# twosixlabs/csl-gan

Hardware: AMD Instinct MI355X
Metric: images/sec/GPU CelebA DCResNet dp_mode=gc bs=128 at 1/2/4/8 MI355X (higher is better)
Workload: dtype f32; 1 GPU; CelebA DCResNet D-step: dp_mode=gc -gcm adaptive-pl -nms 32, WGAN-GP on mean samples, 3x64x64; compute_dtype=fp32_auto, storage_dtype=fp32, launch=hip_graph, batch_per_gpu=128, global_batch=128, parallelism=dp1, materialize=ghost, grad_sample_dtype=fp32, fuse_passes=True

## Files before the change

### csl_gan_amd/DCResNet_models.py

```python
import torch
import torch.nn.functional as F
from torch import nn

from . import functional as HF
from . import ops
from .models import Discriminator, Generator
from .nn import HipConv2d, HipGroupNormAct, HipLinear


class UpsampleConv(nn.Module):

    def __init__(self, in_ch, out_ch, filter_size, bias=True):
        super().__init__()
        self.conv = HipConv2d(in_ch, out_ch, filter_size, padding="same", bias=bias)

    def forward_shuffled(self, x_ps):
        return self.conv.forward_shuffled(x_ps)

    def forward(self, x):
        if x.is_cuda:
            if x.shape[1] % 4:
                raise NotImplementedError("UpsampleConv on HIP needs in_ch %% 4 == 0 (got %d)" % x.shape[1])
            return HF.nchw_view(self.forward_shuffled(HF.DepthToSpace.apply(HF.nhwc(x))))
        return self.conv(F.pixel_shuffle(torch.cat([x, x, x, x], 1), 2))
# ... 39 lines not shown
    from . import nn as hnn
    return (not torch.is_grad_enabled()) and x.is_cuda and x.dtype == torch.float32 and not ops.storage_bf16() and hnn._mask_recorder is None


def _norm_as_affine(norm, x, part, conv):
    if part is None or not ops.in_affine_ok(x, conv.weight.permute(0, 2, 3, 1), conv.stride[0], conv.padding[0]):
        return None
    N, H, W, C = x.shape
    sc, sh = ops.groupnorm_affine(part, norm.weight.detach(), norm.bias.detach(), norm.num_groups, norm.eps, N, H * W, C)
    return sc, sh, bool(norm.relu)


def _norm_act(bn, ch):
    return _BatchNormAct(ch) if bn else HipGroupNormAct(32, ch, relu=True)


class ResBlockUp(nn.Module):

    def __init__(self, in_ch, out_ch, filter_size, bn=True):
        super().__init__()
        self.shortcut = UpsampleConv(in_ch, out_ch, 1)
        self.bn1 = _norm_act(bn, in_ch)
        self.convUp = UpsampleConv(in_ch, out_ch, filter_size, bias=False)
        self.bn2 = _norm_act(bn, out_ch)
        self.conv = HipConv2d(out_ch, out_ch, filter_size, padding="same")

    def forward_nhwc(self, x):
        return self.forward_nhwc_parts(x)[0]

    def forward_nhwc_parts(self, x, x_part=None, next_norm=None):
        if x.shape[-1] % 4:
            raise NotImplementedError("ResBlockUp on HIP needs in_ch %% 4 == 0 (got %d)" % x.shape[-1])
        fuse = _gn_fusable(x)
        a_ps, x_ps = self.bn1.forward_shuffled(x, part=x_part) if x_part is not None else self.bn1.forward_shuffled(x)
        s = self.shortcut.forward_shuffled(x_ps)
        affine = None
        if fuse and isinstance(self.bn2, HipGroupNormAct):
            with ops.gn_partials(self.bn2.num_groups) as cell:
                o = self.convUp.forward_shuffled(a_ps)
            affine = _norm_as_affine(self.bn2, o, cell.part, self.conv)
            h = o if affine is not None else self.bn2.forward_nhwc(o, part=cell.part)
        else:
            h = self.bn2.forward_nhwc(self.convUp.forward_shuffled(a_ps))
        if fuse and isinstance(next_norm, HipGroupNormAct):
            with ops.gn_partials(next_norm.num_groups) as cell:
                out = self.conv.forward_nhwc(h, residual=s, in_affine=affine)
            return out, cell.part
        return self.conv.forward_nhwc(h, residual=s, in_affine=affine), None

    def forward(self, x):
        if x.is_cuda:
            return HF.nchw_view(self.forward_nhwc(HF.nhwc(x)))
        return self.conv(self.bn2(self.convUp(self.bn1(x)))) + self.shortcut(x)


class DCResNetGenerator(Generator):
    def __init__(self, channels, first_filter_size, **kwargs):
        super().__init__(**kwargs)
        self.first_filter_size = first_filter_size
        extra = self.n_classes if self.emb_mode == "concat" else 0
        self.linIn = HipLinear(self.z_dim + extra, first_filter_size ** 2 * channels[0])
        self.blocks = nn.ModuleList([ResBlockUp(a, b, 5, bn=self.bn) for a, b in zip(channels[:-1], channels[1:])])
        self.bn = _norm_act(self.bn, channels[-1])
        self.convOut = HipConv2d(channels[-1], self.out_ch, 3, padding="same", act=ops.ACT_TANH)

    def forward(self, z, y=None, out=None):
        f = self.first_filter_size
        x = self.linIn(self._condition(z, y)).reshape(z.size(0), -1, f, f)
# ... 70 lines not shown
```

### csl_gan_amd/_lib.py

```python
from __future__ import annotations

import ctypes as C
import os

_HERE = os.path.dirname(os.path.abspath(__file__))
LIB_PATH = os.environ.get("CSLGAN_LIB_PATH") or os.path.join(_HERE, "libcslgan_hip.so")
MAX_SEGS = 16
ABI_VERSION = 7

EXPORTS = [
    "cslgan_version", "cslgan_last_error", "cslgan_last_kernel", "cslgan_device_count",
    "cslgan_sample_sqnorm_f32", "cslgan_sample_sqnorm_bf16", "cslgan_clip_factors_f32", "cslgan_clip_accum_noise_f32",
    "cslgan_clip_accum_noise_bf16", "cslgan_conv2d_wgrad_grouped_bf16out_f32",
    "cslgan_l2_clip_rows_f32", "cslgan_row_l2norm_f32", "cslgan_row_l2norm_bwd_f32", "cslgan_mean_sample_f32",
    "cslgan_conv2d_fwd_f32", "cslgan_conv2d_fwd_x3_f32", "cslgan_conv2d_dgrad_f32", "cslgan_conv2d_wgrad_grouped_f32",
    "cslgan_conv2d_wgrad_scaled_f32", "cslgan_conv2d_wgrad_blocks_f32", "cslgan_conv2d_wgrad_sqnorm_gram_f32", "cslgan_conv2d_wgrad_skinny_f32", "cslgan_conv2d_s2_fwd_f32",
    "cslgan_conv2d_dgrad_x3_f32", "cslgan_conv2d_s2_fwd_x3_f32", "cslgan_u8_to_f32_nhwc", "cslgan_split_filter_x3_f32",
    "cslgan_depth_to_space_f32", "cslgan_fold_channels4_f32",
    "cslgan_bias_grad_grouped_f32", "cslgan_act_bwd_f32", "cslgan_groupnorm_act_f32", "cslgan_groupnorm_apply_parts_f32", "cslgan_groupnorm_affine_parts_f32", "cslgan_batchnorm_act_f32", "cslgan_batchnorm_eval_act_f32",
    "cslgan_norm_act_bwd_f32", "cslgan_norm_bwd_ws_floats",
    "cslgan_adam_step_f32", "cslgan_adam_step_dev_f32", "cslgan_adam_multi_f32",
    "cslgan_adaptive_clip_f32", "cslgan_segment_means_f32", "cslgan_segment_means_bwd_f32", "cslgan_dstep_stats_f32", "cslgan_grad_log_stats_f32",
    "cslgan_lerp_rows_f32", "cslgan_lipschitz_term_f32", "cslgan_lipschitz_term_bwd_f32",
    "cslgan_conv2d_fwd_bf16s", "cslgan_conv2d_dgrad_bf16s", "cslgan_conv2d_wgrad_grouped_bf16s", "cslgan_cast_f32_bf16", "cslgan_cast_bf16_f32",
    "cslgan_act_bwd_bf16", "cslgan_bias_grad_grouped_bf16", "cslgan_linear_k1_dgrad_bf16s", "cslgan_linear_k1_wgrad_bf16s",
    "cslgan_conv2d_c3_fwd_bf16out", "cslgan_conv2d_c3_wgrad_bf16gy", "cslgan_groupnorm_act_bf16s",
    "cslgan_conv2d_fwd_skinny_bf16in", "cslgan_conv2d_dgrad_skinny_bf16in", "cslgan_conv2d_wgrad_scaled_bf16s",
    "cslgan_latent_normal_f32", "cslgan_f32_to_u8",
    "cslgan_attack_trials", "cslgan_rank_counts", "cslgan_softmax_max_rows_f32",
    "cslgan_ovr_logreg_ws_floats", "cslgan_ovr_logreg_eval_f32", "cslgan_ovr_logreg_proba_f32",
    "cslgan_ovr_logreg_u8_ws_floats", "cslgan_ovr_logreg_eval_u8", "cslgan_ovr_logreg_proba_u8",
    "cslgan_ovr_mlp_u8_ws_floats", "cslgan_ovr_mlp_eval_u8", "cslgan_ovr_mlp_proba_u8",
    "cslgan_class_moments_u8", "cslgan_nb_score_gauss_u8", "cslgan_nb_score_bern_u8",
    "cslgan_nn_padded_dim", "cslgan_nn_prepare_u8", "cslgan_nn_min_i8", "cslgan_nn_count_i8",
    "cslgan_nn_kth_workspace_bytes", "cslgan_nn_kth_i8", "cslgan_nn_count_radius_i8",
]


class SegsT(C.Structure):
    _fields_ = [
        ("n_seg", C.c_int32), ("_pad", C.c_int32),
        ("inp", C.c_void_p * MAX_SEGS), ("out", C.c_void_p * MAX_SEGS), ("noise", C.c_void_p * MAX_SEGS),
        ("len", C.c_int64 * MAX_SEGS), ("row_stride", C.c_int64 * MAX_SEGS), ("rows", C.c_int64 * MAX_SEGS), ("call_counter", C.c_void_p),
    ]


MAX_CLIP_LAYERS, MAX_CLIP_JOBS = 32, 16


class AdaptiveClipT(C.Structure):
    _fields_ = [
        ("n_layers", C.c_int32), ("n_mat", C.c_int32), ("n_jobs", C.c_int32), ("_pad", C.c_int32),
# ... 30 lines not shown
    vp, i32, i64, f32, u64 = C.c_void_p, C.c_int, C.c_int64, C.c_float, C.c_uint64
    sig = {
        "cslgan_version": [],
        "cslgan_device_count": [],
        "cslgan_sample_sqnorm_f32": [C.POINTER(SegsT), i64, vp, vp],
        "cslgan_sample_sqnorm_bf16": [C.POINTER(SegsT), i64, vp, vp],
        "cslgan_clip_accum_noise_bf16": [C.POINTER(SegsT), i64, vp, i32, vp, u64, u64, f32, f32, vp],
        "cslgan_conv2d_wgrad_grouped_bf16out_f32": [C.POINTER(ConvT), vp, vp, i32, f32, vp, vp, vp],
        "cslgan_clip_factors_f32": [vp, i32, i64, vp, i32, f32, i64, vp, vp, vp],
        "cslgan_clip_accum_noise_f32": [C.POINTER(SegsT), i64, vp, i32, vp, u64, u64, f32, f32, vp],
        "cslgan_l2_clip_rows_f32": [vp, vp, i64, i64, f32, vp, vp],
        "cslgan_mean_sample_f32": [vp, i32, i32, i64, vp, vp, i64, f32, f32, u64, u64, vp, vp, vp],
        "cslgan_row_l2norm_f32": [vp, i64, i64, vp, vp],
        "cslgan_row_l2norm_bwd_f32": [vp, vp, vp, i64, i64, vp, vp],
        "cslgan_conv2d_fwd_f32": [C.POINTER(ConvT), vp, vp, vp, vp, i32, vp, vp],
        "cslgan_conv2d_fwd_x3_f32": [C.POINTER(ConvT), vp, vp, vp, i32, vp, vp, i32, vp, vp],
        "cslgan_conv2d_dgrad_f32": [C.POINTER(ConvT), vp, vp, vp, i32, vp, vp, vp],
        "cslgan_conv2d_dgrad_x3_f32": [C.POINTER(ConvT), vp, vp, vp, vp, i32, vp, vp, vp],
        "cslgan_norm_act_bwd_f32": [vp, vp, vp, vp, vp, i64, i64, i32, i32, f32, i32, vp, vp, vp, vp, vp],
        "cslgan_depth_to_space_f32": [vp, i32, i32, i32, i32, i32, vp, vp],
        "cslgan_fold_channels4_f32": [vp, i64, i32, i32, vp, vp],
        "cslgan_conv2d_wgrad_grouped_f32": [C.POINTER(ConvT), vp, vp, i32, f32, vp, vp, vp],
        "cslgan_conv2d_wgrad_scaled_f32": [C.POINTER(ConvT), vp, vp, vp, i32, f32, vp, vp],
        "cslgan_conv2d_wgrad_blocks_f32": [C.POINTER(ConvT), vp, vp, f32, i32, C.POINTER(C.c_int32), C.POINTER(vp), C.POINTER(vp), vp],
        "cslgan_conv2d_wgrad_sqnorm_gram_f32": [C.POINTER(ConvT), vp, vp, f32, vp, vp],
        "cslgan_conv2d_wgrad_skinny_f32": [C.POINTER(ConvT), vp, vp, f32, vp, i32, vp],
        "cslgan_conv2d_s2_fwd_f32": [C.POINTER(ConvT), vp, vp, vp, i32, vp, i32, vp, vp],
        "cslgan_conv2d_s2_fwd_x3_f32": [C.POINTER(ConvT), vp, vp, vp, vp, i32, vp, i32, vp, vp],
        "cslgan_bias_grad_grouped_f32": [vp, i32, i32, i32, i32, f32, vp, vp, vp],
        "cslgan_act_bwd_f32": [vp, vp, i64, f32, vp, vp],
        "cslgan_groupnorm_act_f32": [vp, vp, vp, i32, i32, i32, i32, f32, i32, vp, vp, i32, vp, vp, vp],
        "cslgan_groupnorm_affine_parts_f32": [vp, i32, vp, vp, i32, i32, i32, i32, f32, vp, vp, vp],
        "cslgan_groupnorm_apply_parts_f32": [vp, vp, vp, i32, i32, i32, i32, f32, i32, vp, i32, vp, vp, i32, vp, vp],
        "cslgan_batchnorm_act_f32": [vp, vp, vp, i64, i32, f32, i32, f32, vp, vp, vp, vp, i64, i32, vp, vp, vp],
        "cslgan_batchnorm_eval_act_f32": [vp, vp, vp, vp, vp, i64, i32, f32, i32, vp, vp, i64, i32, vp, vp],
        "cslgan_adam_step_f32": [vp, vp, vp, vp, i64, f32, f32, f32, f32, f32, i32, vp],
        "cslgan_adam_step_dev_f32": [vp, vp, vp, vp, i64, f32, f32, f32, f32, f32, vp, vp],
        "cslgan_adam_multi_f32": [i32, C.POINTER(vp), C.POINTER(vp), C.POINTER(vp), C.POINTER(vp), C.POINTER(i64), f32, f32, f32, f32, f32,
                                  i32, vp, vp],
        "cslgan_adaptive_clip_f32": [C.POINTER(AdaptiveClipT), i64, i64, i32, f32, i32, f32, i64, vp, vp, vp, vp, vp, vp],
        "cslgan_segment_means_f32": [vp, i32, C.POINTER(C.c_int32), C.POINTER(f32), vp, vp, vp],
        "cslgan_segment_means_bwd_f32": [vp, vp, i32, C.POINTER(C.c_int32), C.POINTER(f32), vp, vp],
        "cslgan_dstep_stats_f32": [vp, i32, vp, i32, vp, vp, vp, vp, vp],
        "cslgan_grad_log_stats_f32": [vp, i32, i64, i64, i32, vp, i32, f32, vp, vp, vp, vp, vp, vp],
        "cslgan_lerp_rows_f32": [vp, vp, vp, i64, i64, vp, vp],
        "cslgan_lipschitz_term_f32": [vp, i64, i64, i32, f32, vp, vp, vp, vp, vp],
        "cslgan_lipschitz_term_bwd_f32": [vp, vp, vp, vp, i64, i64, i32, f32, vp, vp],
        "cslgan_conv2d_fwd_bf16s": [C.POINTER(ConvT), vp, vp, vp, i32, vp, vp, i32, i32, vp, i32, vp],
        "cslgan_conv2d_dgrad_bf16s": [C.POINTER(ConvT), vp, vp, vp, i32, vp, vp, i32, vp],
        "cslgan_conv2d_wgrad_grouped_bf16s": [C.POINTER(ConvT), vp, vp, i32, f32, vp, i32, vp, vp],
        "cslgan_cast_f32_bf16": [vp, vp, i64, vp],
        "cslgan_u8_to_f32_nhwc": [vp, vp, i32, i32, i32, i32, C.c_float, C.c_float, vp, vp],
        "cslgan_split_filter_x3_f32": [vp, i32, i32, i32, vp, i32, vp],
        "cslgan_cast_bf16_f32": [vp, vp, i64, vp],
        "cslgan_act_bwd_bf16": [vp, vp, i64, f32, vp, vp],
        "cslgan_bias_grad_grouped_bf16": [vp, i32, i32, i32, i32, f32, vp, vp, vp],
        "cslgan_linear_k1_dgrad_bf16s": [vp, vp, vp, i32, i64, vp, vp],
        "cslgan_linear_k1_wgrad_bf16s": [vp, vp, vp, i32, i64, i32, f32, vp, vp, vp],
        "cslgan_conv2d_wgrad_scaled_bf16s": [C.POINTER(ConvT), vp, vp, vp, i32, f32, vp, vp],
        "cslgan_conv2d_c3_fwd_bf16out": [C.POINTER(ConvT), vp, vp, vp, i32, vp, vp],
        "cslgan_conv2d_c3_wgrad_bf16gy": [C.POINTER(ConvT), vp, vp, f32, vp, vp, vp],
        "cslgan_groupnorm_act_bf16s": [vp, i32, vp, vp, i32, i32, i32, i32, f32, i32, vp, vp, i32, vp, vp],
        "cslgan_conv2d_fwd_skinny_bf16in": [C.POINTER(ConvT), vp, vp, vp, i32, vp, vp],
        "cslgan_conv2d_dgrad_skinny_bf16in": [C.POINTER(ConvT), vp, vp, vp, i32, vp, vp],
        "cslgan_latent_normal_f32": [u64, u64, vp, i64, i32, vp, i32, i32, vp, vp],
        "cslgan_f32_to_u8": [vp, i64, f32, f32, vp, vp],
# ... 44 lines not shown
```

### csl_gan_amd/build.py

```python
import os
import subprocess
import sys

HERE = os.path.dirname(os.path.abspath(__file__))
CSRC = os.path.join(HERE, "csrc")
LIB = os.path.join(HERE, "libcslgan_hip.so")
SOURCES = ["clip_kernels.hip", "igemm_kc.hip", "igemm_halo.hip", "igemm_skinny.hip", "igemm_mc.hip", "igemm_wgh.hip", "igemm_bf16.hip", "igemm_x3.hip", "igemm_bf16s.hip", "conv_c3.hip", "linear_k1.hip", "conv1x1.hip", "gram_norm.hip", "pointwise_kernels.hip", "step_kernels.hip", "attack_kernels.hip", "logreg_kernels.hip", "mlp_kernels.hip", "nb_kernels.hip", "nn_kernels.hip"]
HEADERS = ["common.h", "igemm.h", "conv_classes.h", "device_prims.h", "kc_frame.h", "ovr_rows.h", os.path.join("..", "..", "include", "cslgan.h")]


def _newer_than(target, deps):
    if not os.path.exists(target):
        return True
    t = os.path.getmtime(target)
    return any(os.path.getmtime(d) > t for d in deps)


def build(force=False, verbose=False):
    force = force or os.environ.get("CSLGAN_FORCE_BUILD", "0") == "1"
    hipcc = os.environ.get("HIPCC", "/opt/rocm/bin/hipcc")
    headers = [os.path.join(CSRC, h) for h in HEADERS]
    objs = []
    procs = []
    os.makedirs(os.path.join(HERE, "build"), exist_ok=True)
    jobs = int(os.environ.get("CSLGAN_BUILD_JOBS", str(min(8, os.cpu_count() or 1))))
    pending = []
    for s in SOURCES:
        o = os.path.join(HERE, "build", s.replace(".hip", ".o"))
        objs.append(o)
        if force or _newer_than(o, [os.path.join(CSRC, s)] + headers):
            pending.append((s, o))
    while pending or procs:
        while pending and len(procs) < jobs:
            s, o = pending.pop(0)
            cmd = [hipcc, "--offload-arch=gfx950", "-O3", "-fPIC", "-std=c++17", "-Wall", "-Wno-unused-function",
                   "-c", os.path.join(CSRC, s), "-o", o]
            if verbose:
                print(" ".join(cmd))
            procs.append((s, subprocess.Popen(cmd, stdout=subprocess.PIPE, stderr=subprocess.STDOUT)))
        s, pr = procs.pop(0)
        out, _ = pr.communicate()
# ... 18 lines not shown
```

### csl_gan_amd/csrc/gram_norm.hip

```cpp
#include "common.h"
#include "device_prims.h"
#include "igemm.h"
#include "conv_classes.h"

namespace cslgan {


struct GramParams {
    const float* gy;
    const float* x;
    int N, H, W, C, K, PQ, Q, T, stride;
    int n1, n2;
    float alpha2;
    float* sq;
    signed char ty[IG_MAX_TAPS], tx[IG_MAX_TAPS];
};

constexpr int GR_LD = 36;

template <int TILES>
__global__ __launch_bounds__(256) void gram_sqnorm_kernel(const GramParams p) {
    constexpr int ROWS = TILES == 1 ? 128 : 64;
    constexpr int LPT = ROWS * 8 / 256;
    __shared__ __attribute__((aligned(16))) float As[2][ROWS * GR_LD];
    __shared__ float s_red[TILES == 1 ? 2 * 1024 : 4];

    const int tid = threadIdx.x;
    const int b = blockIdx.x;
    const int cpc = p.C >> 5;
    const int n_chunks = p.n1 + p.n2;
    const int n_iter = TILES == 1 ? (n_chunks + 3) / 4 : n_chunks;

    int l_pix[LPT], l_slot[LPT], l_py[LPT], l_px[LPT];
    const int j4 = (tid & 7) * 4;
#pragma unroll
    for (int i = 0; i < LPT; ++i) {
        const int row = (tid >> 3) + 32 * i;
        l_slot[i] = TILES == 1 ? row >> 5 : 0;
        l_pix[i] = TILES == 1 ? row & 31 : row;
        l_py[i] = l_pix[i] / p.Q;
        l_px[i] = l_pix[i] - l_py[i] * p.Q;
    }
    constexpr int DEPTH = TILES == 1 ? 4 : 6;
    float4 rg[DEPTH][LPT];
    auto load = [&](int it, float4* dst) {
#pragma unroll
        for (int i = 0; i < LPT; ++i) {
            const int c = TILES == 1 ? 4 * it + l_slot[i] : it;
            float4 v = make_float4(0.f, 0.f, 0.f, 0.f);
            if (l_pix[i] < p.PQ && c < n_chunks) {
                if (c < p.n1) {
                    v = *reinterpret_cast<const float4*>(p.gy + ((long long)b * p.PQ + l_pix[i]) * p.K + c * 32 + j4);
                } else {
                    const int c2 = c - p.n1;
                    const int t = c2 / cpc, cc = c2 - t * cpc;
                    const int iy = l_py[i] * p.stride + p.ty[t], ix = l_px[i] * p.stride + p.tx[t];
                    if ((unsigned)iy < (unsigned)p.H && (unsigned)ix < (unsigned)p.W)
                        v = *reinterpret_cast<const float4*>(p.x + (((long long)b * p.H + iy) * p.W + ix) * p.C + cc * 32 + j4);
// ... 34 lines not shown
                if (c < n_chunks) {
                    float4 af[4], bf[4];
#pragma unroll
                    for (int g = 0; g < 4; ++g) {
                        af[g] = *reinterpret_cast<const float4*>(&As[buf][rowA * GR_LD + 8 * g + 4 * h]);
                        bf[g] = *reinterpret_cast<const float4*>(&As[buf][rowB * GR_LD + 8 * g + 4 * h]);
                    }
                    if (c < p.n1) {
#pragma unroll
                        for (int g = 0; g < 4; ++g) {
                            acc1 = __builtin_amdgcn_mfma_f32_32x32x2f32(af[g].x, bf[g].x, acc1, 0, 0, 0);
                            acc1 = __builtin_amdgcn_mfma_f32_32x32x2f32(af[g].y, bf[g].y, acc1, 0, 0, 0);
                            acc1 = __builtin_amdgcn_mfma_f32_32x32x2f32(af[g].z, bf[g].z, acc1, 0, 0, 0);
                            acc1 = __builtin_amdgcn_mfma_f32_32x32x2f32(af[g].w, bf[g].w, acc1, 0, 0, 0);
                        }
                    } else {
#pragma unroll
                        for (int g = 0; g < 4; ++g) {
                            acc2 = __builtin_amdgcn_mfma_f32_32x32x2f32(af[g].x, bf[g].x, acc2, 0, 0, 0);
                            acc2 = __builtin_amdgcn_mfma_f32_32x32x2f32(af[g].y, bf[g].y, acc2, 0, 0, 0);
                            acc2 = __builtin_amdgcn_mfma_f32_32x32x2f32(af[g].z, bf[g].z, acc2, 0, 0, 0);
                            acc2 = __builtin_amdgcn_mfma_f32_32x32x2f32(af[g].w, bf[g].w, acc2, 0, 0, 0);
                        }
                    }
                }
                buf ^= 1;
            }
        }
    }
    __syncthreads();

    float prod = 0.f;
    if (TILES == 1) {
        for (int i = tid; i < 2 * 1024; i += 256) s_red[i] = 0.f;
        __syncthreads();
#pragma unroll
        for (int v = 0; v < 16; ++v) {
            const int row = (v & 3) + 8 * (v >> 2) + 4 * h;
            atomicAdd(&s_red[row * 32 + r], acc1[v]);
            atomicAdd(&s_red[1024 + row * 32 + r], acc2[v]);
        }
        __syncthreads();
        for (int i = tid; i < 1024; i += 256) prod = fmaf(s_red[i], s_red[1024 + i], prod);
        __syncthreads();
        const float tot = block_sum_256(prod, s_red);
        if (tid == 0) atomicAdd(p.sq + b, p.alpha2 * tot);
    } else {
#pragma unroll
        for (int v = 0; v < 16; ++v) prod = fmaf(acc1[v], acc2[v], prod);
        const float tot = block_sum_256(prod, s_red);
        if (tid == 0) atomicAdd(p.sq + b, p.alpha2 * tot);
    }
}



struct GramSmallParams {
    const float* gy;
    const float* x;
    int N, H, W, C, K, PQ, Q, T, s;
    float alpha2;
    float* sq;
    signed char tcls[IG_MAX_TAPS], tdy[IG_MAX_TAPS], tdx[IG_MAX_TAPS];
    int Hc[4], Wc[4];
};

__global__ __launch_bounds__(256) void gram_sqnorm_small_kernel(const GramSmallParams p) {
    __shared__ float XXs[4][16 * 17];
    __shared__ float G1s[4][16 * 17];
    __shared__ float s_red[4];
    const int tid = threadIdx.x, lane = tid & 63, wid = tid >> 6;
    const int b = blockIdx.x;
    const int row = lane & 15, q = lane >> 4;
    const int nc = p.s * p.s;
    f32x4 accx = {0.f, 0.f, 0.f, 0.f};
    if (wid < nc) {
        const int cy = wid / p.s, cx = wid - cy * p.s;
// ... 231 lines not shown
```

### csl_gan_amd/csrc/pointwise_kernels.hip

```cpp
#include "common.h"
#include "device_prims.h"

namespace cslgan {

__global__ void act_bwd_kernel(const float* __restrict__ g, const float* __restrict__ y, long long n, float slope,
                               float* __restrict__ out, int vec) {
    const long long stride = (long long)gridDim.x * blockDim.x;
    if (vec) {
        const long long n4 = n >> 2;
        const float4* g4 = reinterpret_cast<const float4*>(g);
        const float4* y4 = reinterpret_cast<const float4*>(y);
        float4* o4 = reinterpret_cast<float4*>(out);
        for (long long i = (long long)blockIdx.x * blockDim.x + threadIdx.x; i < n4; i += stride) {
            const float4 a = g4[i], b = y4[i];
            o4[i] = make_float4(b.x > 0.f ? a.x : slope * a.x, b.y > 0.f ? a.y : slope * a.y,
                                b.z > 0.f ? a.z : slope * a.z, b.w > 0.f ? a.w : slope * a.w);
        }
        for (long long i = (n4 << 2) + (long long)blockIdx.x * blockDim.x + threadIdx.x; i < n; i += stride)
            out[i] = y[i] > 0.f ? g[i] : slope * g[i];
    } else {
        for (long long i = (long long)blockIdx.x * blockDim.x + threadIdx.x; i < n; i += stride)
            out[i] = y[i] > 0.f ? g[i] : slope * g[i];
    }
}

constexpr int NS_ROWS_MIN = 64;

typedef unsigned short bf16_t;
__device__ __forceinline__ float ldf(const float* p, long long i) { return p[i]; }
__device__ __forceinline__ float ldf(const bf16_t* p, long long i) { return bf2f(p[i]); }
__device__ __forceinline__ float4 ld4(const float* p, long long i) { return *reinterpret_cast<const float4*>(p + i); }
__device__ __forceinline__ float4 ld4(const bf16_t* p, long long i) {
    const uint2 v = *reinterpret_cast<const uint2*>(p + i);
    return make_float4(bf_lo(v.x), bf_hi(v.x), bf_lo(v.y), bf_hi(v.y));
// ... 144 lines not shown
            const long long s = (i / per_stat_elems) * n_groups + c / cpg;
            const float mean = mean_tab ? mean_tab[s] : stats[2 * s] * inv_cnt;
            const float rstd = rsqrtf(stats[2 * s + 1] * inv_cnt + eps);
            const float xi = ldf(x, i);
            float t = (xi - mean) * rstd * gamma[c] + beta[c];
            t = (relu && t < 0.f) ? 0.f : t;
            if (D2S) {
                const long long off = d2s_offset(i / C, c & 3, H, W, C >> 2) + (c >> 2);
                st1(y, off, t);
                if (xs) st1(xs, off, xi);
            } else {
                st1(y, i, t);
            }
        }
    }
}

template <bool D2S, typename TX, typename TY>
__global__ __launch_bounds__(256) void norm_apply_rows_kernel(const TX* __restrict__ x, const float* __restrict__ gamma, const float* __restrict__ beta,
                                                              const float* __restrict__ stats, long long rows_per_stat, int C, int cpg, int n_groups,
                                                              float eps, int relu, TY* __restrict__ y, int H, int W, TY* __restrict__ xs,
                                                              const float* __restrict__ part, int n_part, float* __restrict__ stats_out, int chan,
                                                              const float* __restrict__ mean_tab) {
    const int c4n = C >> 2;
    const int lg = __ffs(c4n) - 1;
    const int c = (threadIdx.x & (c4n - 1)) << 2;
    const long long sr = blockIdx.y;
    const float cnt = (float)rows_per_stat * (float)cpg;
    const float inv_cnt = 1.f / cnt;
    const long long base = sr * rows_per_stat * C;
    float mean[4], rstd[4], ga[4], be[4];
    if (part) {
        extern __shared__ float s_st[];
        for (int i = threadIdx.x; chan && i < n_groups; i += 256) {
            float sum = 0.f;
            for (int b = 0; b < n_part; ++b) sum += part[((sr * n_part + b) * n_groups + i) * 2];
            const float nb = cnt / (float)n_part, mean_all = sum / cnt;
            float css = 0.f;
            for (int b = 0; b < n_part; ++b) {
                const float* q = part + ((sr * n_part + b) * n_groups + i) * 2;
                const float dm = q[0] / nb - mean_all;
                css += q[1] + nb * dm * dm;
            }
            s_st[2 * i] = mean_all;
            s_st[2 * i + 1] = css;
            if (stats_out && blockIdx.x == 0) {
                stats_out[2 * (sr * n_groups + i)] = sum;
                stats_out[2 * (sr * n_groups + i) + 1] = css;
            }
        }
        for (int i = threadIdx.x; !chan && i < n_groups; i += 256) {
            float S1 = 0.f, S2 = 0.f;
            for (int b = 0; b < n_part; ++b) {
                const float* q = part + ((sr * n_part + b) * n_groups + i) * 2;
                S1 += q[0];
                S2 += q[1];
            }
            const float k = ldf(x, base + (long long)i * cpg);
            const float m1 = S1 / cnt;
            float css = S2 - S1 * m1;
            css = css < 0.f ? 0.f : css;
            s_st[2 * i] = k + m1;
            s_st[2 * i + 1] = css;
            if (stats_out && blockIdx.x == 0) {
                stats_out[2 * (sr * n_groups + i)] = (k + m1) * cnt;
                stats_out[2 * (sr * n_groups + i) + 1] = css;
            }
        }
        __syncthreads();
#pragma unroll
        for (int e = 0; e < 4; ++e) {
            const int g = (c + e) / cpg;
            mean[e] = s_st[2 * g];
            rstd[e] = rsqrtf(s_st[2 * g + 1] * inv_cnt + eps);
        }
    } else {
#pragma unroll
        for (int e = 0; e < 4; ++e) {
            const long long s = sr * n_groups + (c + e) / cpg;
            mean[e] = mean_tab ? mean_tab[s] : stats[2 * s] * inv_cnt;
            rstd[e] = rsqrtf(stats[2 * s + 1] * inv_cnt + eps);
        }
    }
#pragma unroll
    for (int e = 0; e < 4; ++e) {
        ga[e] = gamma[c + e];
        be[e] = beta[c + e];
    }
    const unsigned n4 = (unsigned)((rows_per_stat * C) >> 2);
    const bool per_image = rows_per_stat == (long long)H * W;
    for (unsigned i = blockIdx.x * 256u + threadIdx.x; i < n4; i += gridDim.x * 256u) {
        const long long e0 = base + ((long long)i << 2);
        const float4 v = ld4(x, e0);
        const float in[4] = {v.x, v.y, v.z, v.w};
        float o[4];
#pragma unroll
        for (int e = 0; e < 4; ++e) {
            const float t = (in[e] - mean[e]) * rstd[e] * ga[e] + be[e];
            o[e] = (relu && t < 0.f) ? 0.f : t;
        }
        if (D2S) {
            const unsigned rl = i >> lg;
            const int Cq = C >> 2, cq = c >> 2;
            long long off[4];
            if (per_image) {
                const unsigned h = rl / (unsigned)W, w = rl - h * (unsigned)W;
#pragma unroll
                for (int e = 0; e < 4; ++e) off[e] = (((sr * 2 * H + 2 * h + (e >> 1)) * 2 * W + 2 * w + (e & 1)) * Cq) + cq;
            } else {
#pragma unroll
                for (int e = 0; e < 4; ++e) off[e] = d2s_offset(sr * rows_per_stat + rl, e, H, W, Cq) + cq;
            }
#pragma unroll
            for (int e = 0; e < 4; ++e) {
                st1(y, off[e], o[e]);
                if (xs) st1(xs, off[e], in[e]);
            }
        } else {
            st4(y, e0, o[0], o[1], o[2], o[3]);
        }
    }
}

template <bool INVERSE>
__global__ void depth_to_space_kernel(const float* __restrict__ in, long long rows, int H, int W, int C, float* __restrict__ out) {
    const int Cq = C >> 2;
    const long long n4 = rows * Cq;
    for (long long i = (long long)blockIdx.x * blockDim.x + threadIdx.x; i < n4; i += (long long)gridDim.x * blockDim.x) {
        const long long r = i / Cq;
        const int cq = (int)(i - r * Cq);
        if (INVERSE) {
            float v[4];
#pragma unroll
// ... 576 lines not shown
```

### csl_gan_amd/ops.py

```python
from __future__ import annotations

import ctypes as C
from typing import List, NamedTuple, Optional, Sequence

import torch

from . import _lib
from ._lib import ConvT, SegsT, check

ACT_NONE, ACT_LRELU02, ACT_RELU, ACT_TANH = 0, 1, 2, 3
COMPUTE_F32, COMPUTE_BF16, COMPUTE_BF16X3 = 0, 1, 2

_compute = COMPUTE_F32
_auto = False


def set_compute_dtype(name):
    global _compute, _auto
    if name not in ("fp32", "bf16", "bf16x3", "fp32_auto"):
        raise ValueError("compute dtype must be 'fp32', 'bf16', 'bf16x3' or 'fp32_auto', got %r" % (name,))
    _auto = name == "fp32_auto"
    _compute = {"fp32": COMPUTE_F32, "bf16": COMPUTE_BF16, "bf16x3": COMPUTE_BF16X3, "fp32_auto": COMPUTE_F32}[name]


# ... 1570 lines not shown
    t = _norm_scratch.get(key)
    if t is None or t.numel() < need:
        t = _norm_scratch[key] = torch.empty(max(need, 1 << 16), device=dev, dtype=torch.float32)
    return t


def groupnorm_act(x, gamma, beta, groups, eps=1e-5, relu=True, return_stats=False, d2s=False, want_raw=False, out_dtype=None, part=None):
    if x.dtype == torch.bfloat16 or out_dtype == torch.bfloat16:
        _chk(x, "x", allow_bf16=True); _chk(gamma, "gamma"); _chk(beta, "beta")
        N, H, W, Cc = x.shape
        y, xs, dW = _d2s_out(x, d2s, want_raw, torch.bfloat16)
        ws = torch.empty(2 * N * groups, device=x.device, dtype=torch.float32)
        check(_lib.lib().cslgan_groupnorm_act_bf16s(_p(x), 1 if x.dtype == torch.bfloat16 else 0, _p(gamma), _p(beta), N, H * W, Cc, groups,
                                                    float(eps), 1 if relu else 0, _p(ws), _p(y), dW, _p(xs), _stream()), "groupnorm_act_bf16s")
        out = (y, xs) if want_raw else y
        return (out, ws) if return_stats else out
    _chk(x, "x"); _chk(gamma, "gamma"); _chk(beta, "beta")
    N, H, W, Cc = x.shape
    y, xs, dW = _d2s_out(x, d2s, want_raw)
    ws = torch.empty(2 * N * groups, device=x.device, dtype=torch.float32)
    if part is not None:
        pt, n_part = part
        check(_lib.lib().cslgan_groupnorm_apply_parts_f32(_p(x), _p(gamma), _p(beta), N, H * W, Cc, groups, float(eps), 1 if relu else 0,
                                                          _p(pt), n_part, _p(ws), _p(y), dW, _p(xs), _stream()), "groupnorm_apply_parts")
        out = (y, xs) if want_raw else y
        return (out, ws) if return_stats else out
    sc = _scratch(x.device, 2 * N * groups)
    check(_lib.lib().cslgan_groupnorm_act_f32(_p(x), _p(gamma), _p(beta), N, H * W, Cc, groups, float(eps), 1 if relu else 0,
                                              _p(ws), _p(y), dW, _p(xs), _p(sc), _stream()), "groupnorm_act")
    out = (y, xs) if want_raw else y
    return (out, ws) if return_stats else out


def batchnorm_act(x, gamma, beta, running_mean=None, running_var=None, momentum=0.1, eps=1e-5, relu=True, return_stats=False,
                  d2s=False, want_raw=False):
    _chk(x, "x"); _chk(gamma, "gamma"); _chk(beta, "beta")
    Cc = x.shape[-1]
    rows = x.numel() // Cc
    if d2s:
        y, xs, dW = _d2s_out(x, d2s, want_raw)
        rpi = x.shape[1] * x.shape[2]
    else:
        y, xs, dW, rpi = torch.empty_like(x), None, 0, 0
    ws = torch.empty(2 * Cc, device=x.device, dtype=torch.float32)
    check(_lib.lib().cslgan_batchnorm_act_f32(_p(x), _p(gamma), _p(beta), rows, Cc, float(eps), 1 if relu else 0, float(momentum),
                                              _p(running_mean), _p(running_var), _p(ws), _p(y), rpi, dW, _p(xs),
                                              _p(_scratch(x.device, 2 * Cc)), _stream()), "batchnorm_act")
    out = (y, xs) if want_raw else y
    return (out, ws) if return_stats else out


def batchnorm_eval_act(x, gamma, beta, running_mean, running_var, eps=1e-5, relu=True, d2s=False, want_raw=False):
    for t, n in ((x, "x"), (gamma, "gamma"), (beta, "beta"), (running_mean, "running_mean"), (running_var, "running_var")):
        _chk(t, n)
    Cc = x.shape[-1]
    rows = x.numel() // Cc
    if d2s:
        y, xs, dW = _d2s_out(x, d2s, want_raw)
        rpi = x.shape[1] * x.shape[2]
    else:
        y, xs, dW, rpi = torch.empty_like(x), None, 0, 0
    ws = torch.empty(2 * Cc, device=x.device, dtype=torch.float32)
    check(_lib.lib().cslgan_batchnorm_eval_act_f32(_p(x), _p(gamma), _p(beta), _p(running_mean), _p(running_var), rows, Cc, float(eps),
                                                   1 if relu else 0, _p(ws), _p(y), rpi, dW, _p(xs), _stream()), "batchnorm_eval_act")
    return (y, xs) if want_raw else y

# ... 127 lines not shown
```

### include/cslgan.h

```cpp
#ifndef CSLGAN_H
#define CSLGAN_H

#include <stdint.h>

#ifdef __cplusplus
extern "C" {
#endif

#define CSLGAN_ABI_VERSION 7

typedef enum {
    CSLGAN_OK = 0,
    CSLGAN_ERR_INVALID_ARG = -1,
    CSLGAN_ERR_LAUNCH = -2,
    CSLGAN_ERR_NO_DEVICE = -3
} cslgan_status;

enum { CSLGAN_ACT_NONE = 0, CSLGAN_ACT_LRELU02 = 1, CSLGAN_ACT_RELU = 2, CSLGAN_ACT_TANH = 3 };

#define CSLGAN_MAX_SEGS 16
#define CSLGAN_MAX_ROLES 8

typedef struct {
    int32_t n_seg;
// ... 122 lines not shown

int cslgan_groupnorm_act_bf16s(const void* x, int x_bf16, const float* gamma, const float* beta, int N, int HW, int C, int groups,
                               float eps, int relu, float* stats_ws, void* y_bf16, int d2s_W, void* x_shuffled_bf16, void* stream);

int cslgan_conv2d_fwd_skinny_bf16in(const cslgan_conv_t* p, const void* x_bf16, const float* w, const float* bias, int act, float* y,
                                    void* stream);
int cslgan_conv2d_dgrad_skinny_bf16in(const cslgan_conv_t* p, const void* gy_bf16, const float* w, float* wt_ws, int repack, float* gx,
                                      void* stream);

int cslgan_conv2d_wgrad_scaled_bf16s(const cslgan_conv_t* p, const void* gy, const void* x, const float* row_scale, int group, float alpha,
                                     float* gw, void* stream);

int cslgan_cast_f32_bf16(const float* in, void* out_bf16, int64_t n, void* stream);
int cslgan_cast_bf16_f32(const void* in_bf16, float* out, int64_t n, void* stream);

int cslgan_act_bwd_bf16(const void* g, const void* y, int64_t n, float slope, void* out, void* stream);
int cslgan_bias_grad_grouped_bf16(const void* gy, int N, int PQ, int K, int group, float alpha, float* gb, float* sq, void* stream);


int cslgan_act_bwd_f32(const float* g, const float* y, int64_t n, float slope, float* out, void* stream);

int cslgan_depth_to_space_f32(const float* in, int N, int H, int W, int C, int inverse, float* out, void* stream);
int cslgan_fold_channels4_f32(const float* in, int64_t rows, int C, int unfold, float* out, void* stream);

#define CSLGAN_NORM_PARTIAL_BLOCKS 64
int cslgan_groupnorm_affine_parts_f32(const float* part, int n_part, const float* gamma, const float* beta, int N, int HW, int C, int groups,
                                      float eps, float* scale, float* shift, void* stream);
int cslgan_groupnorm_apply_parts_f32(const float* x, const float* gamma, const float* beta, int N, int HW, int C, int groups,
                                     float eps, int relu, const float* part, int n_part, float* stats_ws, float* y, int d2s_W,
                                     float* x_shuffled, void* stream);
int cslgan_groupnorm_act_f32(const float* x, const float* gamma, const float* beta, int N, int HW, int C,
                             int groups, float eps, int relu, float* stats_ws, float* y, int d2s_W, float* x_shuffled,
                             float* scratch, void* stream);

int cslgan_batchnorm_act_f32(const float* x, const float* gamma, const float* beta, int64_t rows, int C, float eps,
                             int relu, float momentum, float* running_mean, float* running_var, float* stats_ws,
                             float* y, int64_t rows_per_image, int d2s_W, float* x_shuffled, float* scratch ,
                             void* stream);

int cslgan_batchnorm_eval_act_f32(const float* x, const float* gamma, const float* beta, const float* running_mean,
                                  const float* running_var, int64_t rows, int C, float eps, int relu, float* stats_ws,
                                  float* y, int64_t rows_per_image, int d2s_W, float* x_shuffled, void* stream);

int cslgan_norm_act_bwd_f32(const float* x, const float* dy, const float* y, const float* gamma, const float* stats,
                            int64_t rows, int64_t rows_per_stat, int C, int groups, float eps, int relu, float* ws,
                            float* dx, float* dgamma, float* dbeta, void* stream);
int64_t cslgan_norm_bwd_ws_floats(int64_t rows, int64_t rows_per_stat, int C, int groups);

int cslgan_adam_step_f32(float* p, const float* g, float* m, float* v, int64_t n, float lr, float b1,
                         float b2, float eps, float weight_decay, int step, void* stream);
int cslgan_adam_step_dev_f32(float* p, const float* g, float* m, float* v, int64_t n, float lr, float b1,
                             float b2, float eps, float weight_decay, const int32_t* step_dev, void* stream);

int cslgan_adam_multi_f32(int n_seg, float* const* p, const float* const* g, float* const* m, float* const* v, const int64_t* n,
                          float lr, float b1, float b2, float eps, float weight_decay, int step, const int32_t* step_dev,
                          void* stream);

int cslgan_segment_means_f32(const float* x, int n_seg, const int32_t* sizes, const float* scale, float* vec, float* total,
                             void* stream);
int cslgan_segment_means_bwd_f32(const float* g_total, const float* g_vec, int n_seg, const int32_t* sizes, const float* scale,
                                 float* gx, void* stream);
int cslgan_dstep_stats_f32(const float* d_real, int n_real, const float* d_fake, int n_fake, const float* real_loss,
                           const float* fake_loss, const float* penalty, float* acc7, void* stream);
int cslgan_grad_log_stats_f32(const float* sq, int n_layers, int64_t ld, int64_t col0, int B, const float* max_norm, int per_layer,
                              float eps, float* acc_mean, float* acc_std, float* acc_max, float* acc_c, float* acc_clipped,
                              void* stream);
// ... 79 lines not shown
```

Before: 20080 images/sec.

## Fuse group-norm apply with 1x1 upsample shortcut conv in generator blocks

Adds an MFMA kernel that applies group norm plus ReLU with depth-to-space to the block input and, in the same pass, computes the 1x1 shortcut conv on the raw shuffled input. This avoids materialising the shuffled raw tensor and launching a separate shortcut conv. Separately, the gram-norm reduction now writes per-wavefront partials into reused staging shared memory instead of doing shared-memory atomics. The fused path only runs in no-grad generator forward with group norm, which may not be on the D-step hot path.

```diff
diff --git a/csl_gan_amd/DCResNet_models.py b/csl_gan_amd/DCResNet_models.py
--- a/csl_gan_amd/DCResNet_models.py
+++ b/csl_gan_amd/DCResNet_models.py
@@ -95,8 +95,16 @@
         if x.shape[-1] % 4:
             raise NotImplementedError("ResBlockUp on HIP needs in_ch %% 4 == 0 (got %d)" % x.shape[-1])
         fuse = _gn_fusable(x)
-        a_ps, x_ps = self.bn1.forward_shuffled(x, part=x_part) if x_part is not None else self.bn1.forward_shuffled(x)
-        s = self.shortcut.forward_shuffled(x_ps)
+        sc = self.shortcut.conv
+        if (fuse and isinstance(self.bn1, HipGroupNormAct) and sc.kernel_size == (1, 1) and sc.act == ops.ACT_NONE and sc._bpc is None
+                and ops.gn_shortcut_ok(x, sc.out_channels, x_part)):
+            w = sc.weight.permute(0, 2, 3, 1).contiguous()
+            a_ps, s = ops.groupnorm_apply_shortcut(x, self.bn1.weight.detach(), self.bn1.bias.detach(), self.bn1.num_groups, x_part,
+                                                   ops.fold_channels4(w.detach(), wkey=sc._wkey(w)),
+                                                   None if sc.bias is None else sc.bias.detach(), eps=self.bn1.eps, relu=self.bn1.relu)
+        else:
+            a_ps, x_ps = self.bn1.forward_shuffled(x, part=x_part) if x_part is not None else self.bn1.forward_shuffled(x)
+            s = self.shortcut.forward_shuffled(x_ps)
         affine = None
         if fuse and isinstance(self.bn2, HipGroupNormAct):
             with ops.gn_partials(self.bn2.num_groups) as cell:
diff --git a/csl_gan_amd/_lib.py b/csl_gan_amd/_lib.py
--- a/csl_gan_amd/_lib.py
+++ b/csl_gan_amd/_lib.py
@@ -17,7 +17,7 @@
     "cslgan_conv2d_wgrad_scaled_f32", "cslgan_conv2d_wgrad_blocks_f32", "cslgan_conv2d_wgrad_sqnorm_gram_f32", "cslgan_conv2d_wgrad_skinny_f32", "cslgan_conv2d_s2_fwd_f32",
     "cslgan_conv2d_dgrad_x3_f32", "cslgan_conv2d_s2_fwd_x3_f32", "cslgan_u8_to_f32_nhwc", "cslgan_split_filter_x3_f32",
     "cslgan_depth_to_space_f32", "cslgan_fold_channels4_f32",
-    "cslgan_bias_grad_grouped_f32", "cslgan_act_bwd_f32", "cslgan_groupnorm_act_f32", "cslgan_groupnorm_apply_parts_f32", "cslgan_groupnorm_affine_parts_f32", "cslgan_batchnorm_act_f32", "cslgan_batchnorm_eval_act_f32",
+    "cslgan_bias_grad_grouped_f32", "cslgan_act_bwd_f32", "cslgan_groupnorm_act_f32", "cslgan_groupnorm_apply_parts_f32", "cslgan_groupnorm_apply_parts_shortcut_f32", "cslgan_groupnorm_affine_parts_f32", "cslgan_batchnorm_act_f32", "cslgan_batchnorm_eval_act_f32",
     "cslgan_norm_act_bwd_f32", "cslgan_norm_bwd_ws_floats",
     "cslgan_adam_step_f32", "cslgan_adam_step_dev_f32", "cslgan_adam_multi_f32",
     "cslgan_adaptive_clip_f32", "cslgan_segment_means_f32", "cslgan_segment_means_bwd_f32", "cslgan_dstep_stats_f32", "cslgan_grad_log_stats_f32",
@@ -114,6 +114,7 @@
         "cslgan_groupnorm_act_f32": [vp, vp, vp, i32, i32, i32, i32, f32, i32, vp, vp, i32, vp, vp, vp],
         "cslgan_groupnorm_affine_parts_f32": [vp, i32, vp, vp, i32, i32, i32, i32, f32, vp, vp, vp],
         "cslgan_groupnorm_apply_parts_f32": [vp, vp, vp, i32, i32, i32, i32, f32, i32, vp, i32, vp, vp, i32, vp, vp],
+        "cslgan_groupnorm_apply_parts_shortcut_f32": [vp, vp, vp, i32, i32, i32, i32, f32, i32, vp, i32, vp, vp, i32, vp, vp, i32, vp, vp],
         "cslgan_batchnorm_act_f32": [vp, vp, vp, i64, i32, f32, i32, f32, vp, vp, vp, vp, i64, i32, vp, vp, vp],
         "cslgan_batchnorm_eval_act_f32": [vp, vp, vp, vp, vp, i64, i32, f32, i32, vp, vp, i64, i32, vp, vp],
         "cslgan_adam_step_f32": [vp, vp, vp, vp, i64, f32, f32, f32, f32, f32, i32, vp],
diff --git a/csl_gan_amd/build.py b/csl_gan_amd/build.py
--- a/csl_gan_amd/build.py
+++ b/csl_gan_amd/build.py
@@ -5,8 +5,8 @@
 HERE = os.path.dirname(os.path.abspath(__file__))
 CSRC = os.path.join(HERE, "csrc")
 LIB = os.path.join(HERE, "libcslgan_hip.so")
-SOURCES = ["clip_kernels.hip", "igemm_kc.hip", "igemm_halo.hip", "igemm_skinny.hip", "igemm_mc.hip", "igemm_wgh.hip", "igemm_bf16.hip", "igemm_x3.hip", "igemm_bf16s.hip", "conv_c3.hip", "linear_k1.hip", "conv1x1.hip", "gram_norm.hip", "pointwise_kernels.hip", "step_kernels.hip", "attack_kernels.hip", "logreg_kernels.hip", "mlp_kernels.hip", "nb_kernels.hip", "nn_kernels.hip"]
-HEADERS = ["common.h", "igemm.h", "conv_classes.h", "device_prims.h", "kc_frame.h", "ovr_rows.h", os.path.join("..", "..", "include", "cslgan.h")]
+SOURCES = ["clip_kernels.hip", "igemm_kc.hip", "igemm_halo.hip", "igemm_skinny.hip", "igemm_mc.hip", "igemm_wgh.hip", "igemm_bf16.hip", "igemm_x3.hip", "igemm_bf16s.hip", "conv_c3.hip", "linear_k1.hip", "conv1x1.hip", "gn_shortcut.hip", "gram_norm.hip", "pointwise_kernels.hip", "step_kernels.hip", "attack_kernels.hip", "logreg_kernels.hip", "mlp_kernels.hip", "nb_kernels.hip", "nn_kernels.hip"]
+HEADERS = ["common.h", "igemm.h", "conv_classes.h", "device_prims.h", "gn_apply.h", "kc_frame.h", "ovr_rows.h", os.path.join("..", "..", "include", "cslgan.h")]
 
 
 def _newer_than(target, deps):
diff --git a/csl_gan_amd/csrc/gn_apply.h b/csl_gan_amd/csrc/gn_apply.h
--- /dev/null
+++ b/csl_gan_amd/csrc/gn_apply.h
@@ -0,0 +1,37 @@
+#pragma once
+#include "common.h"
+
+namespace cslgan {
+
+__device__ __forceinline__ void gn_combine_chan(const float* __restrict__ part, long long sr, int n_part, int n_groups, float cnt,
+                                                float* s_st, float* __restrict__ stats_out, bool publish) {
+    for (int i = threadIdx.x; i < n_groups; i += 256) {
+        float sum = 0.f;
+        for (int b = 0; b < n_part; ++b) sum += part[((sr * n_part + b) * n_groups + i) * 2];
+        const float nb = cnt / (float)n_part, mean_all = sum / cnt;
+        float css = 0.f;
+        for (int b = 0; b < n_part; ++b) {
+            const float* q = part + ((sr * n_part + b) * n_groups + i) * 2;
+            const float dm = q[0] / nb - mean_all;
+            css += q[1] + nb * dm * dm;
+        }
+        s_st[2 * i] = mean_all;
+        s_st[2 * i + 1] = css;
+        if (stats_out && publish) {
+            stats_out[2 * (sr * n_groups + i)] = sum;
+            stats_out[2 * (sr * n_groups + i) + 1] = css;
+        }
+    }
+}
+
+__device__ __forceinline__ void gn_group_stat(const float* s_st, int g, float inv_cnt, float eps, float& mean, float& rstd) {
+    mean = s_st[2 * g];
+    rstd = rsqrtf(s_st[2 * g + 1] * inv_cnt + eps);
+}
+
+__device__ __forceinline__ float gn_apply(float x, float mean, float rstd, float ga, float be, int relu) {
+    const float t = (x - mean) * rstd * ga + be;
+    return (relu && t < 0.f) ? 0.f : t;
+}
+
+}
diff --git a/csl_gan_amd/csrc/gn_shortcut.hip b/csl_gan_amd/csrc/gn_shortcut.hip
--- /dev/null
+++ b/csl_gan_amd/csrc/gn_shortcut.hip
@@ -0,0 +1,173 @@
+#include "common.h"
+#include "device_prims.h"
+#include "gn_apply.h"
+
+namespace cslgan {
+
+constexpr int GS_MAX_GROUPS = 256;
+
+struct GsParams {
+    const float* x;
+    const float* gamma;
+    const float* beta;
+    const float* part;
+    const float* wf;
+    const float* bias;
+    float* stats;
+    float* a_ps;
+    float* s;
+    int HW, W, cpg, n_groups, n_part, K, relu, tiles;
+    float eps;
+};
+
+template <int CQ, int TR>
+__global__ __launch_bounds__(256, CQ == 32 ? 4 : 2) void gn_shortcut_kernel(const GsParams p) {
+    constexpr int LD = CQ + 4, C = 4 * CQ, ROWS = 4 * TR;
+    constexpr int RSTEP = 256 / CQ, AREG = TR / RSTEP;
+    constexpr int WREG = 64 * (CQ / 4) / 256;
+    constexpr int NT = TR == 32 ? 2 : 1;
+    __shared__ __attribute__((aligned(16))) float As[ROWS * LD];
+    __shared__ __attribute__((aligned(16))) float Ws[64 * LD];
+    __shared__ int s_row[ROWS];
+    __shared__ float s_st[2 * GS_MAX_GROUPS];
+
+    const int tid = threadIdx.x, lane = tid & 63, wid = tid >> 6;
+    const int r = lane & 31, h = lane >> 5;
+    const int cq = tid & (CQ - 1), rl0 = tid / CQ;
+    const long long n = blockIdx.y;
+    const float cnt = (float)p.HW * (float)p.cpg;
+    const float inv_cnt = 1.f / cnt;
+    gn_combine_chan(p.part, n, p.n_part, p.n_groups, cnt, s_st, p.stats, blockIdx.x == 0);
+    __syncthreads();
+    float mean[4], rstd[4], ga[4], be[4];
+#pragma unroll
+    for (int e = 0; e < 4; ++e) {
+        gn_group_stat(s_st, (4 * cq + e) / p.cpg, inv_cnt, p.eps, mean[e], rstd[e]);
+        ga[e] = p.gamma[4 * cq + e];
+        be[e] = p.beta[4 * cq + e];
+    }
+    const float* xi = p.x + n * p.HW * C;
+    float* ai = p.a_ps + n * p.HW * C;
+    float* si = p.s + n * 4 * p.HW * p.K;
+    const int W = p.W;
+    const int arow = (TR == 32 ? wid : (wid & 1)) * 32;
+    const int fo = TR == 32 ? 0 : (wid >> 1) * 32;
+
+    float4 ra[AREG];
+    f32x4 rw[WREG];
+    float rb[NT], bv[NT];
+    auto fetch = [&](int tile) {
+#pragma unroll
+        for (int j = 0; j < AREG; ++j)
+            ra[j] = *reinterpret_cast<const float4*>(xi + (size_t)(tile * TR + rl0 + j * RSTEP) * C + 4 * cq);
+    };
+    auto fetch_w = [&](int n0) {
+#pragma unroll
+        for (int j = 0; j < WREG; ++j) {
+            const int idx = tid + 256 * j;
+            rw[j] = *reinterpret_cast<const f32x4*>(p.wf + (size_t)(n0 + idx / (CQ / 4)) * CQ + (idx % (CQ / 4)) * 4);
+        }
+#pragma unroll
+        for (int j = 0; j < NT; ++j) rb[j] = p.bias ? p.bias[n0 + fo + j * 32 + r] : 0.f;
+    };
+    const int first = blockIdx.x;
+    if (first < p.tiles) {
+        fetch(first);
+        fetch_w(0);
+    }
+    for (int tile = first; tile < p.tiles; tile += gridDim.x) {
+        __syncthreads();
+        if (tid < ROWS) {
+            const unsigned rl = tile * TR + (tid % TR), hh = rl / (unsigned)W, ww = rl - hh * (unsigned)W;
+            const int ij = tid / TR;
+            s_row[tid] = (2 * hh + (ij >> 1)) * 2 * W + 2 * ww + (ij & 1);
+        }
+#pragma unroll
+        for (int j = 0; j < AREG; ++j) {
+            const int row = rl0 + j * RSTEP;
+            const unsigned rl = tile * TR + row, hh = rl / (unsigned)W, ww = rl - hh * (unsigned)W;
+            const float in[4] = {ra[j].x, ra[j].y, ra[j].z, ra[j].w};
+#pragma unroll
+            for (int e = 0; e < 4; ++e) {
+                As[(e * TR + row) * LD + cq] = in[e];
+                ai[(size_t)((2 * hh + (e >> 1)) * 2 * W + 2 * ww + (e & 1)) * CQ + cq] = gn_apply(in[e], mean[e], rstd[e], ga[e], be[e], p.relu);
+            }
+        }
+        if (tile + (int)gridDim.x < p.tiles) fetch(tile + gridDim.x);
+        for (int n0 = 0; n0 < p.K; n0 += 64) {
+            if (n0) __syncthreads();
+#pragma unroll
+            for (int j = 0; j < WREG; ++j) {
+                const int idx = tid + 256 * j;
+                *reinterpret_cast<f32x4*>(&Ws[(idx / (CQ / 4)) * LD + (idx % (CQ / 4)) * 4]) = rw[j];
+            }
+#pragma unroll
+            for (int j = 0; j < NT; ++j) bv[j] = rb[j];
+            fetch_w(n0 + 64 < p.K ? n0 + 64 : 0);
+            __syncthreads();
+            f32x16 acc[NT];
+#pragma unroll
+            for (int j = 0; j < NT; ++j)
+#pragma unroll
+                for (int v = 0; v < 16; ++v) acc[j][v] = 0.f;
+#pragma unroll 4
+            for (int g = 0; g < CQ / 8; ++g) {
+                const float4 a = *reinterpret_cast<const float4*>(&As[(arow + r) * LD + 8 * g + 4 * h]);
+#pragma unroll
+                for (int j = 0; j < NT; ++j) {
+                    const float4 b = *reinterpret_cast<const float4*>(&Ws[(fo + j * 32 + r) * LD + 8 * g + 4 * h]);
+                    acc[j] = __builtin_amdgcn_mfma_f32_32x32x2f32(a.x, b.x, acc[j], 0, 0, 0);
+                    acc[j] = __builtin_amdgcn_mfma_f32_32x32x2f32(a.y, b.y, acc[j], 0, 0, 0);
+                    acc[j] = __builtin_amdgcn_mfma_f32_32x32x2f32(a.z, b.z, acc[j], 0, 0, 0);
+                    acc[j] = __builtin_amdgcn_mfma_f32_32x32x2f32(a.w, b.w, acc[j], 0, 0, 0);
+                }
+            }
+#pragma unroll
+            for (int j = 0; j < NT; ++j) {
+                const int f = n0 + fo + j * 32 + r;
+#pragma unroll
+                for (int v = 0; v < 16; ++v)
+                    si[s_row[arow + 4 * h + (v & 3) + 8 * (v >> 2)] * p.K + f] = acc[j][v] + bv[j];
+            }
+        }
+    }
+}
+
+template <int CQ, int TR>
+static int launch_gn_shortcut(GsParams& p, int N, int per_cu, hipStream_t st) {
+    p.tiles = p.HW / TR;
+    int gx = 256 * per_cu / N;
+    gx = gx < 1 ? 1 : (gx > p.tiles ? p.tiles : gx);
+    const int walk = (p.tiles + gx - 1) / gx;
+    gx = (p.tiles + walk - 1) / walk;
+    note_kernel("gn_shortcut_kernel<%d>", CQ);
+    hipLaunchKernelGGL((gn_shortcut_kernel<CQ, TR>), dim3((unsigned)gx, (unsigned)N), dim3(256), 0, st, p);
+    return check_launch("gn_shortcut_kernel");
+}
+
+}
+
+using namespace cslgan;
+
+extern "C" int cslgan_groupnorm_apply_parts_shortcut_f32(const float* x, const float* gamma, const float* beta, int N, int HW, int C, int groups,
+                                                         float eps, int relu, const float* part, int n_part, float* stats_ws, float* y,
+                                                         int d2s_W, const float* wf, const float* bias, int K, float* s, void* stream) {
+    CSLGAN_REQUIRE(x && gamma && beta && part && stats_ws && y && wf && s, "groupnorm_apply_parts_shortcut: null argument");
+    CSLGAN_REQUIRE(N > 0 && HW > 0 && C > 0 && C % 4 == 0, "groupnorm_apply_parts_shortcut: needs C %% 4 == 0 (C=%d)", C);
+    CSLGAN_REQUIRE(groups > 0 && groups <= GS_MAX_GROUPS && C % groups == 0,
+                   "groupnorm_apply_parts_shortcut: C=%d not divisible by groups=%d (at most %d groups)", C, groups, GS_MAX_GROUPS);
+    CSLGAN_REQUIRE(C == 128 || C == 256 || C == 512, "groupnorm_apply_parts_shortcut: C / 4 must be 32, 64 or 128 (C=%d)", C);
+    CSLGAN_REQUIRE(K >= 64 && K % 64 == 0, "groupnorm_apply_parts_shortcut: K=%d is not a multiple of 64", K);
+    CSLGAN_REQUIRE(N <= 65535 && n_part >= 1 && n_part <= CSLGAN_NORM_PARTIAL_BLOCKS && HW == 64 * n_part,
+                   "groupnorm_apply_parts_shortcut: needs HW == 64 * n_part <= %d * 64 (n_part=%d)", CSLGAN_NORM_PARTIAL_BLOCKS, n_part);
+    CSLGAN_REQUIRE(d2s_W > 0 && HW % d2s_W == 0, "groupnorm_apply_parts_shortcut: d2s_W=%d does not divide the %d pixels of an image", d2s_W, HW);
+    CSLGAN_REQUIRE(4ll * HW * K < (1ll << 31), "groupnorm_apply_parts_shortcut: image of %d x %d outputs too large", 4 * HW, K);
+    CSLGAN_REQUIRE(aligned16(x) && aligned16(y) && aligned16(wf) && aligned16(s), "groupnorm_apply_parts_shortcut: misaligned pointer");
+    GsParams p{};
+    p.x = x; p.gamma = gamma; p.beta = beta; p.part = part; p.wf = wf; p.bias = bias; p.stats = stats_ws; p.a_ps = y; p.s = s;
+    p.HW = HW; p.W = d2s_W; p.cpg = C / groups; p.n_groups = groups; p.n_part = n_part; p.K = K; p.relu = relu; p.eps = eps;
+    hipStream_t st = (hipStream_t)stream;
+    if (C == 128) return launch_gn_shortcut<32, 32>(p, N, 4, st);
+    if (C == 256) return launch_gn_shortcut<64, 32>(p, N, 2, st);
+    return launch_gn_shortcut<128, 16>(p, N, 2, st);
+}
diff --git a/csl_gan_amd/csrc/gram_norm.hip b/csl_gan_amd/csrc/gram_norm.hip
--- a/csl_gan_amd/csrc/gram_norm.hip
+++ b/csl_gan_amd/csrc/gram_norm.hip
@@ -23,7 +23,8 @@
     constexpr int ROWS = TILES == 1 ? 128 : 64;
     constexpr int LPT = ROWS * 8 / 256;
     __shared__ __attribute__((aligned(16))) float As[2][ROWS * GR_LD];
-    __shared__ float s_red[TILES == 1 ? 2 * 1024 : 4];
+    __shared__ float s_red[4];
+    static_assert(TILES != 1 || 2 * ROWS * GR_LD >= 4 * 2048, "the staging buffers hold the four wavefronts' partial matrices");
 
     const int tid = threadIdx.x;
     const int b = blockIdx.x;
@@ -124,17 +125,19 @@
 
     float prod = 0.f;
     if (TILES == 1) {
-        for (int i = tid; i < 2 * 1024; i += 256) s_red[i] = 0.f;
-        __syncthreads();
+        float* red = &As[0][0];
 #pragma unroll
         for (int v = 0; v < 16; ++v) {
             const int row = (v & 3) + 8 * (v >> 2) + 4 * h;
-            atomicAdd(&s_red[row * 32 + r], acc1[v]);
-            atomicAdd(&s_red[1024 + row * 32 + r], acc2[v]);
+            red[wid * 2048 + row * 32 + r] = acc1[v];
+            red[wid * 2048 + 1024 + row * 32 + r] = acc2[v];
         }
         __syncthreads();
-        for (int i = tid; i < 1024; i += 256) prod = fmaf(s_red[i], s_red[1024 + i], prod);
-        __syncthreads();
+        for (int i = tid; i < 1024; i += 256) {
+            const float g1 = ((red[i] + red[2048 + i]) + red[4096 + i]) + red[6144 + i];
+            const float g2 = ((red[1024 + i] + red[3072 + i]) + red[5120 + i]) + red[7168 + i];
+            prod = fmaf(g1, g2, prod);
+        }
         const float tot = block_sum_256(prod, s_red);
         if (tid == 0) atomicAdd(p.sq + b, p.alpha2 * tot);
     } else {
diff --git a/csl_gan_amd/csrc/pointwise_kernels.hip b/csl_gan_amd/csrc/pointwise_kernels.hip
--- a/csl_gan_amd/csrc/pointwise_kernels.hip
+++ b/csl_gan_amd/csrc/pointwise_kernels.hip
@@ -1,5 +1,6 @@
 #include "common.h"
 #include "device_prims.h"
+#include "gn_apply.h"
 
 namespace cslgan {
 
@@ -210,23 +211,7 @@
     float mean[4], rstd[4], ga[4], be[4];
     if (part) {
         extern __shared__ float s_st[];
-        for (int i = threadIdx.x; chan && i < n_groups; i += 256) {
-            float sum = 0.f;
-            for (int b = 0; b < n_part; ++b) sum += part[((sr * n_part + b) * n_groups + i) * 2];
-            const float nb = cnt / (float)n_part, mean_all = sum / cnt;
-            float css = 0.f;
-            for (int b = 0; b < n_part; ++b) {
-                const float* q = part + ((sr * n_part + b) * n_groups + i) * 2;
-                const float dm = q[0] / nb - mean_all;
-                css += q[1] + nb * dm * dm;
-            }
-            s_st[2 * i] = mean_all;
-            s_st[2 * i + 1] = css;
-            if (stats_out && blockIdx.x == 0) {
-                stats_out[2 * (sr * n_groups + i)] = sum;
-                stats_out[2 * (sr * n_groups + i) + 1] = css;
-            }
-        }
+        if (chan) gn_combine_chan(part, sr, n_part, n_groups, cnt, s_st, stats_out, blockIdx.x == 0);
         for (int i = threadIdx.x; !chan && i < n_groups; i += 256) {
             float S1 = 0.f, S2 = 0.f;
             for (int b = 0; b < n_part; ++b) {
@@ -248,9 +233,7 @@
         __syncthreads();
 #pragma unroll
         for (int e = 0; e < 4; ++e) {
-            const int g = (c + e) / cpg;
-            mean[e] = s_st[2 * g];
-            rstd[e] = rsqrtf(s_st[2 * g + 1] * inv_cnt + eps);
+            gn_group_stat(s_st, (c + e) / cpg, inv_cnt, eps, mean[e], rstd[e]);
         }
     } else {
 #pragma unroll
@@ -273,10 +256,7 @@
         const float in[4] = {v.x, v.y, v.z, v.w};
         float o[4];
 #pragma unroll
-        for (int e = 0; e < 4; ++e) {
-            const float t = (in[e] - mean[e]) * rstd[e] * ga[e] + be[e];
-            o[e] = (relu && t < 0.f) ? 0.f : t;
-        }
+        for (int e = 0; e < 4; ++e) o[e] = gn_apply(in[e], mean[e], rstd[e], ga[e], be[e], relu);
         if (D2S) {
             const unsigned rl = i >> lg;
             const int Cq = C >> 2, cq = c >> 2;
diff --git a/csl_gan_amd/ops.py b/csl_gan_amd/ops.py
--- a/csl_gan_amd/ops.py
+++ b/csl_gan_amd/ops.py
@@ -1626,6 +1626,39 @@
     return (out, ws) if return_stats else out
 
 
+_GN_SHORTCUT_FUSE = True
+
+
+def gn_shortcut_ok(x, K, part):
+    if not (_GN_SHORTCUT_FUSE and part is not None and x.is_cuda and x.dtype == torch.float32 and x.dim() == 4):
+        return False
+    N, H, W, Cc = x.shape
+    return Cc in (128, 256, 512) and K >= 64 and K % 64 == 0 and N <= 65535 and H * W == 64 * part[1] and 4 * H * W * K < 2 ** 31
+
+
+def groupnorm_apply_shortcut(x, gamma, beta, groups, part, wf, bias=None, eps=1e-5, relu=True, return_stats=False):
+    _chk(x, "x"); _chk(gamma, "gamma"); _chk(beta, "beta"); _chk(wf, "wf")
+    N, H, W, Cc = x.shape
+    K = wf.shape[0]
+    if wf.numel() != K * (Cc // 4):
+        raise RuntimeError("groupnorm_apply_shortcut: wf must be [K, 1, 1, C/4] = [%d, 1, 1, %d]" % (K, Cc // 4))
+    if bias is not None:
+        _chk(bias, "bias")
+        if bias.numel() != K:
+            raise RuntimeError("groupnorm_apply_shortcut: bias must have K = %d elements" % K)
+    pt, n_part = part
+    a_ps = torch.empty((N, 2 * H, 2 * W, Cc // 4), device=x.device, dtype=torch.float32)
+    s = torch.empty((N, 2 * H, 2 * W, K), device=x.device, dtype=torch.float32)
+    ws = torch.empty(2 * N * groups, device=x.device, dtype=torch.float32)
+    rows = 4 * N * H * W
+    _timed("groupnorm_apply_shortcut", 2.0 * rows * K * Cc, 4.0 * (2 * N * H * W * Cc + wf.numel() + rows * K),
+           lambda: check(_lib.lib().cslgan_groupnorm_apply_parts_shortcut_f32(
+               _p(x), _p(gamma), _p(beta), N, H * W, Cc, groups, float(eps), 1 if relu else 0, _p(pt), n_part, _p(ws), _p(a_ps), W,
+               _p(wf), _p(bias), K, _p(s), _stream()), "groupnorm_apply_parts_shortcut"),
+           exec_flop=2.0 * rows * K * (Cc // 4), tag=lambda: "N%d %dx%d C%d K%d" % (N, H, W, Cc, K))
+    return (a_ps, s, ws) if return_stats else (a_ps, s)
+
+
 def batchnorm_act(x, gamma, beta, running_mean=None, running_var=None, momentum=0.1, eps=1e-5, relu=True, return_stats=False,
                   d2s=False, want_raw=False):
     _chk(x, "x"); _chk(gamma, "gamma"); _chk(beta, "beta")
diff --git a/include/cslgan.h b/include/cslgan.h
--- a/include/cslgan.h
+++ b/include/cslgan.h
@@ -178,6 +178,9 @@
 int cslgan_groupnorm_act_f32(const float* x, const float* gamma, const float* beta, int N, int HW, int C,
                              int groups, float eps, int relu, float* stats_ws, float* y, int d2s_W, float* x_shuffled,
                              float* scratch, void* stream);
+int cslgan_groupnorm_apply_parts_shortcut_f32(const float* x, const float* gamma, const float* beta, int N, int HW, int C, int groups,
+                                              float eps, int relu, const float* part, int n_part, float* stats_ws, float* y,
+                                              int d2s_W, const float* wf, const float* bias, int K, float* s, void* stream);
 
 int cslgan_batchnorm_act_f32(const float* x, const float* gamma, const float* beta, int64_t rows, int C, float eps,
                              int relu, float momentum, float* running_mean, float* running_var, float* stats_ws,
```

Result: faster. 20460 images/sec, median of 6 (+1.9%).
